# BigCiLeng/bilateral-driving

Hardware: AMD Instinct MI355X
Metric: train iters/sec (fwd+bwd) at 2M Gaussians, 6x1920x1080; HBM roofline % (higher is better)
Workload: dtype f32

## Files before the change

### bilateral_driving_amd/_lib.py

```python
from __future__ import annotations

import ctypes as C
import os
import threading

import torch

_HERE = os.path.dirname(os.path.abspath(__file__))
LIB_PATH = os.environ.get("BDS_LIB") or os.path.join(_HERE, "libbds.so")
ABI_VERSION = 6

_lock = threading.Lock()
_lib = None

_f = C.c_void_p
_i, _i64, _sz, _fl = C.c_int, C.c_int64, C.c_size_t, C.c_float


class BdsLevel(C.Structure):

    _fields_ = [("grid", C.c_void_p), ("v_grid", C.c_void_p), ("gx", C.c_int32), ("gy", C.c_int32), ("gl", C.c_int32),
                ("factor", C.c_int32), ("n_avg", C.c_int32)]


# ... 12 lines not shown
    "bds_abi_version": (C.c_int, []),
    "bds_strerror": (C.c_char_p, [_i]),
    "bds_set_option": (_i, [_i, _i]),
    "bds_get_option": (_i, [_i]),
    "bds_timer_create": (C.c_void_p, []),
    "bds_timer_destroy": (_i, [_f]),
    "bds_timer_mark": (_i, [_f, _f]),
    "bds_timer_elapsed_ms": (C.c_float, [_f, _f]),
    "bds_last_hip_error": (_i, []),
    "bds_sh_fwd": (_i, [_i64, _i, _i, _f, _f, _f, _f, _f]),
    "bds_sh_bwd": (_i, [_i64, _i, _i, _f, _f, _f, _f, _f, _f, _f]),
    "bds_project_fwd": (_i, [_i, _i64, _f, _f, _f, _f, _f, _f, _i, _i, _fl, _fl, _fl, _fl, _f, _f, _f, _f, _f, _f, _f]),
    "bds_project_bwd": (_i, [_i, _i64, _f, _f, _f, _f, _f, _i, _i, _fl, _f, _f, _f, _f, _f, _f, _f, _f, _f, _f, _f, _f]),
    "bds_isect_prepare_workspace_bytes": (_sz, [_i, _i64]),
    "bds_isect_visible_ids_offset": (_sz, [_i, _i64]),
    "bds_isect_build_workspace_bytes": (_sz, [_i, _i64, _i64]),
    "bds_isect_prepare": (_i, [_i, _i64, _f, _f, _f, _f, _f, _i, _i, _i, _f, _f, _sz, _i64, _i64, _f, _f, _i, _f]),
    "bds_isect_build": (_i, [_i, _i64, _i64, _i64, _f, _f, _f, _f, _f, _i, _i, _i, _f, _sz, _f, _sz, _f, _f, _f, _f, _i, _i, _f]),
    "bds_isect_tiles": (_i, [_i, _i64, _f, _f, _f, _f, _f, _i, _i, _i, _f, _f, _sz, _f, _sz, _i64, _f, _f, _f, C.POINTER(C.c_int64),
                             C.POINTER(C.c_int64), _f]),
    "bds_splat_pack_rgbd": (_i, [_i64, _f, _f, _f, _f, _f, _f, _f, _f, _f]),
    "bds_expected_depth_fwd": (_i, [_i64, _f, _f, _f, _f]),
    "bds_expected_depth_bwd": (_i, [_i64, _i, _i, _f, _f, _f, _f, _f, _f, _f]),
    "bds_expected_depth_split_fwd": (_i, [_i64, _i, _f, _f, _f, _f, _f]),
    "bds_expected_depth_split_bwd": (_i, [_i64, _i, _f, _f, _f, _f, _f, _f, _f, _f]),
    "bds_splat_pack": (_i, [_i64, _f, _i, _f, _f, _f, _f, _f, _f, _f, _f, _f, _i64, _f, _f]),
    "bds_rasterize_fwd": (_i, [_i, _i64, _i64, _f, _i, _f, _f, _i, _i, _i, _i, _i, _i, _f, _f, _f, _f, _f, _f, _f, _i, _i, _i64, _f]),
    "bds_rasterize_bwd": (_i, [_i, _i64, _i64, _f, _i, _f, _f, _i, _i, _i, _i, _i, _i, _f, _f, _f, _f, _f, _f, _f, _f, _i, _f, _i, _i, _i64, _f]),
    "bds_rasterize_kernel_name": (_i, [_i, _i, _i, _i, C.c_char_p, _i]),
    "bds_rasterize_bwd_schedule": (_i, [_i, _i, _i, _i, _i, _i, _i, _f, _f, _f, _f]),
    "bds_project_view_fwd": (_i, [_i, _i64, _f, _f, _f, _f, _f, _f, _i, _i, _fl, _fl, _fl, _fl, _f, _f, _f, _f, _f, _f, _f, _f, _f, _sz, _f, _f]),
    "bds_gaussian_block_bounds": (_i, [_i64, _f, _f, _f, _f]),
    "bds_sh_view_fwd": (_i, [_i64, _i, _i, _f, _f, _f, _f, _f, _f, _f, _f]),
    "bds_sh_view_bwd_list": (_i, [_i64, _f, _f, _i, _i, _f, _f, _f, _i, _f, _f, _f, _f, _i, _f]),
    "bds_splat_pack_sh": (_i, [_i64, _f, _f, _i, _i, _f, _f, _f, _f, _f, _f, _f, _f, _f, _f, _f, _f, _f, _i64, _f, _f]),
    "bds_nonfinite_flags": (_i, [_i, _f, _f, _f, _f, _f, _f]),
    "bds_project_view_bwd_list": (_i, [_i, _i64, _f, _f, _f, _f, _f, _f, _f, _f, _i, _i, _fl, _f, _f, _f, _f, _f, _f, _f, _f, _f, _f, _f]),
    "bds_view_grads_clear_list": (_i, [_i64, _f, _f, _i, _f, _f, _f, _f, _f, _f, _f, _f]),
    "bds_view_grads_add_list": (_i, [_i64, _f, _i, _f, _f, _f, _f, _f, _f, _f, _f, _f, _f, _f]),
    "bds_isect_counts_offset": (_sz, [_i]),
    "bds_rasterize_schedule_ints": (_i64, [_i, _i, _i]),
    "bds_rasterize_split_pool_ints": (_i64, [_i, _i, _i, _i, _i64, _i64]),
    "bds_rasterize_bwd_schedule_sort": (_i, [_i, _i, _i, _f, _f]),
    "bds_union_slots_workspace_bytes": (_sz, [_i64]),
    "bds_union_slots": (_i, [_i64, _f, _i64, _i, _f, _f, _f, _f, _f, _f, _f, _f, _sz, _f, _f, _f]),
    "bds_bilagrid_slice_fwd": (_i, [_i64, _f, _i, _i, _i, _f, _f, _f, _f]),
# ... 247 lines not shown
```

### bilateral_driving_amd/csrc/project.hip

```cpp
#include "bds_common.h"
#include "gs_math.h"

namespace bds {

constexpr int kProjBlock = 256;

template <bool kAA = false>
__global__ __launch_bounds__(kProjBlock) void project_fwd_kernel(
    int C, int64_t N, const float *__restrict__ means, const float *__restrict__ quats, const float *__restrict__ scales,
    const float *__restrict__ viewmats, const float *__restrict__ Ks, int W, int H, float eps2d, float near_plane,
    float far_plane, float radius_clip, int32_t *__restrict__ radii, float *__restrict__ means2d,
    float *__restrict__ depths, float *__restrict__ conics, float *__restrict__ comps,
    const float *__restrict__ opacities = nullptr, float *__restrict__ opac_eff = nullptr) {
  const int64_t g = (int64_t)blockIdx.x * kProjBlock + threadIdx.x;
  if (g >= N) return;
  float m[3] = {means[g * 3], means[g * 3 + 1], means[g * 3 + 2]};
  float q[4] = {quats[g * 4], quats[g * 4 + 1], quats[g * 4 + 2], quats[g * 4 + 3]};
  float s[3] = {scales[g * 3], scales[g * 3 + 1], scales[g * 3 + 2]};
  const float op = (kAA && opacities) ? opacities[g] : 0.f;
  for (int c = 0; c < C; c++) {
    Camera cam = load_camera(viewmats + c * 16, Ks + c * 9);
    Proj p = project_one(m, q, s, cam, W, H, eps2d, near_plane, far_plane, radius_clip, kAA);
    const int64_t o = (int64_t)c * N + g;
    radii[o] = p.radius;
// ... 63 lines not shown
    }
  }
  if (live) {
    for (int i = 0; i < 3; i++) { v_means[g * 3 + i] = am[i]; v_scales[g * 3 + i] = as[i]; }
    for (int i = 0; i < 4; i++) v_quats[g * 4 + i] = aq[i];
  }
}

template <bool kReduce, bool kAA = false>
__global__ __launch_bounds__(kProjBlock) void project_view_fwd_kernel(
    int64_t N, const float *__restrict__ means, const float *__restrict__ quats, const float *__restrict__ log_scales,
    const float *__restrict__ logits, const float *__restrict__ viewmat, const float *__restrict__ K, int W, int H,
    float eps2d, float near_plane, float far_plane, float radius_clip, float *__restrict__ scales,
    float *__restrict__ opacities, int32_t *__restrict__ radii, float *__restrict__ means2d, float *__restrict__ depths,
    float *__restrict__ conics, PrepReduceSlots rs, int32_t *__restrict__ tiles_per_gauss, int rows,
    const float *__restrict__ block_bounds, float *__restrict__ opac_eff = nullptr) {
  const int64_t g = (int64_t)blockIdx.x * kProjBlock + threadIdx.x;
  if (kReduce) {
    if (blockIdx.x == 0 && threadIdx.x == 0) *rs.m_total = 0;
    for (int64_t i = g; i < rs.zero_elems; i += (int64_t)gridDim.x * kProjBlock) rs.zero_me[i] = 0u;
  }
  if (block_bounds != nullptr) {
    const float *bb = block_bounds + (int64_t)blockIdx.x * 8;
    const float lo[3] = {bb[0], bb[1], bb[2]}, hi[3] = {bb[4], bb[5], bb[6]};
    if (!box_may_be_visible(lo, hi, bb[3], load_camera(viewmat, K), W, H, eps2d, near_plane, far_plane)) {
      if (g < N) {
        radii[g] = 0;
        scales[g * 3] = 0.f; scales[g * 3 + 1] = 0.f; scales[g * 3 + 2] = 0.f; opacities[g] = 0.f;
        if (rows) {
          float4 *row = reinterpret_cast<float4 *>(means2d + g * 8);
          row[0] = row[1] = make_float4(0.f, 0.f, 0.f, 0.f);
        } else {
          means2d[g * 2] = 0.f; means2d[g * 2 + 1] = 0.f;
          depths[g] = 0.f;
          conics[g * 3] = 0.f; conics[g * 3 + 1] = 0.f; conics[g * 3 + 2] = 0.f;
          if (kAA) opac_eff[g] = 0.f;
        }
        if (kReduce && tiles_per_gauss) tiles_per_gauss[g] = 0;
      }
      if (kReduce && threadIdx.x == 0) rs.sums256[blockIdx.x] = 0u;
      return;
    }
  }
  if (kReduce) {
    int radius = 0;
    if (g < N) {
      float m[3] = {means[g * 3], means[g * 3 + 1], means[g * 3 + 2]};
      float q[4] = {quats[g * 4], quats[g * 4 + 1], quats[g * 4 + 2], quats[g * 4 + 3]};
      float s[3];
#pragma unroll
      for (int k = 0; k < 3; k++) {
        s[k] = expf(log_scales[g * 3 + k]);
        scales[g * 3 + k] = s[k];
      }
      const float op = 1.f / (1.f + expf(-logits[g]));
// ... 4 lines not shown
      radii[g] = p.radius;
      const float oe = kAA ? op * p.comp : op;
      if (rows) {
        float4 *row = reinterpret_cast<float4 *>(means2d + g * 8);
        row[0] = make_float4(p.mx, p.my, p.depth, __int_as_float(p.radius));
        row[1] = make_float4(p.ca, p.cb, p.cc, oe);
      } else {
        means2d[g * 2] = p.mx; means2d[g * 2 + 1] = p.my;
        depths[g] = p.depth;
        conics[g * 3] = p.ca; conics[g * 3 + 1] = p.cb; conics[g * 3 + 2] = p.cc;
        if (kAA) opac_eff[g] = oe;
      }
      if (tiles_per_gauss) tiles_per_gauss[g] = 0;
    }
    const int cnt = __syncthreads_count(radius > 0);
    if (threadIdx.x == 0) rs.sums256[blockIdx.x] = (uint32_t)cnt;
    return;
  }
  if (g >= N) return;
  float m[3] = {means[g * 3], means[g * 3 + 1], means[g * 3 + 2]};
  float q[4] = {quats[g * 4], quats[g * 4 + 1], quats[g * 4 + 2], quats[g * 4 + 3]};
  float s[3];
#pragma unroll
  for (int k = 0; k < 3; k++) {
    s[k] = expf(log_scales[g * 3 + k]);
    scales[g * 3 + k] = s[k];
  }
  const float op = 1.f / (1.f + expf(-logits[g]));
  opacities[g] = op;
  Camera cam = load_camera(viewmat, K);
  Proj p = project_one(m, q, s, cam, W, H, eps2d, near_plane, far_plane, radius_clip, kAA);
  radii[g] = p.radius;
  const float oe = kAA ? op * p.comp : op;
// ... 197 lines not shown
  else
    hipLaunchKernelGGL(project_bwd_kernel<false>, dim3((unsigned)cdiv(N, kProjBlock)), dim3(kProjBlock), 0, as_stream(stream), C, N,
                       means, quats, scales, viewmats, Ks, W, H, eps2d, radii, v_means2d, v_depths, v_conics, v_means,
                       v_quats, v_scales, v_viewmats, static_cast<const float *>(nullptr));
  BDS_LAUNCH_CHECK();
  return BDS_OK;
}

static int view_rows(const float *means2d, const float *depths, const float *conics, int *rows) {
  const bool a = depths == means2d + 2, b = conics == means2d + 4;
  if (a != b || (a && !aligned16(means2d))) return BDS_EINVAL;
  *rows = a ? 1 : 0;
  return BDS_OK;
}

extern "C" int bds_project_view_fwd(int flags, int64_t N, const float *means, const float *quats, const float *log_scales,
                                    const float *logits, const float *viewmat, const float *K, int W, int H, float eps2d, float near_plane,
                                    float far_plane, float radius_clip, float *scales, float *opacities, float *opac_eff, int32_t *radii,
                                    float *means2d, float *depths, float *conics, int32_t *tiles_per_gauss, void *prep_ws,
                                    size_t prep_ws_bytes, const float *block_bounds, bds_stream_t stream) {
  BDS_REQUIRE((flags & ~BDS_PROJ_ANTIALIASED) == 0 && N >= 0 && W > 0 && H > 0);
  BDS_REQUIRE(prep_ws == nullptr || N > 0);
  if (N == 0) return BDS_OK;
  BDS_REQUIRE(means && quats && log_scales && logits && viewmat && K && scales && opacities && radii && means2d && depths && conics);
  int rows = 0;
  if (view_rows(means2d, depths, conics, &rows) != BDS_OK) return BDS_EINVAL;
  const bool aa = flags & BDS_PROJ_ANTIALIASED;
  BDS_REQUIRE(aa ? (rows || opac_eff) : opac_eff == nullptr);
  static_assert(kProjBlock == 256, "the tile stage reads the visible counts per 256 Gaussians");
  PrepReduceSlots rs{};
  if (prep_ws) {
    int rc = prep_reduce_slots(prep_ws, prep_ws_bytes, N, &rs);
    if (rc != BDS_OK) return rc;
  } else {
    tiles_per_gauss = nullptr;
  }
  const dim3 grid((unsigned)cdiv(N, kProjBlock)), block(kProjBlock);
#define BDS_VIEW_FWD(R, A)                                                                                                            \
  hipLaunchKernelGGL((project_view_fwd_kernel<R, A>), grid, block, 0, as_stream(stream), N, means, quats, log_scales, logits, viewmat, \
                     K, W, H, eps2d, near_plane, far_plane, radius_clip, scales, opacities, radii, means2d, depths, conics, rs,         \
                     tiles_per_gauss, rows, block_bounds, opac_eff)
  if (prep_ws) { if (aa) BDS_VIEW_FWD(true, true); else BDS_VIEW_FWD(true, false); }
  else         { if (aa) BDS_VIEW_FWD(false, true); else BDS_VIEW_FWD(false, false); }
#undef BDS_VIEW_FWD
  BDS_LAUNCH_CHECK();
  return BDS_OK;
}

namespace bds {
__global__ __launch_bounds__(kProjBlock) void block_bounds_kernel(int64_t N, const float *__restrict__ means,
                                                                 const float *__restrict__ log_scales, float *__restrict__ bounds) {
  __shared__ float red[kProjBlock / kWave][8];
  const int64_t g = (int64_t)blockIdx.x * kProjBlock + threadIdx.x;
  float v[7] = {3.0e38f, 3.0e38f, 3.0e38f, -3.0e38f, -3.0e38f, -3.0e38f, -3.0e38f};
  if (g < N) {
    for (int k = 0; k < 3; k++) { const float m = means[g * 3 + k]; v[k] = m; v[3 + k] = m; }
    v[6] = fmaxf(fmaxf(log_scales[g * 3], log_scales[g * 3 + 1]), log_scales[g * 3 + 2]);
    if (!(v[0] == v[0]) || !(v[1] == v[1]) || !(v[2] == v[2]) || !(v[6] == v[6])) {
      for (int k = 0; k < 3; k++) { v[k] = -3.0e38f; v[3 + k] = 3.0e38f; }
      v[6] = 80.f;
    }
// ... 91 lines not shown
```

### bilateral_driving_amd/csrc/tiles.hip

```cpp
#include "bds_common.h"
#include "gs_math.h"

namespace bds {

constexpr int kScanBlock = 256;
constexpr int kScanItems = 8;
constexpr int kScanTile = kScanBlock * kScanItems;

__device__ __forceinline__ uint32_t wave_incl_scan(uint32_t v) {
  const int lane = threadIdx.x & (kWave - 1);
#pragma unroll
  for (int o = 1; o < kWave; o <<= 1) {
    uint32_t t = __shfl_up(v, o);
    if (lane >= o) v += t;
  }
  return v;
}

__device__ __forceinline__ uint32_t block_excl_scan(uint32_t v, uint32_t &total, uint32_t *lds_w ) {
  const int lane = threadIdx.x & (kWave - 1), wv = threadIdx.x / kWave;
  const int nw = blockDim.x / kWave;
  uint32_t inc = wave_incl_scan(v);
  if (lane == kWave - 1) lds_w[wv] = inc;
  __syncthreads();
// ... 713 lines not shown
  if (threadIdx.x == 0) tile_sums[blockIdx.x] = tot;
}

constexpr int kCompactSpan = kScanTile / kShortChunk + 1;
struct VisCompactSh {
  uint32_t lw[kScanBlock / kWave + 1];
  uint32_t h[kCompactSpan][256];
};
__device__ __forceinline__ void visible_compact_block(VisCompactSh &sh, int vb, int nvb, int64_t CN, const int32_t *radii, const float *depths,
                                                      const uint32_t *tile_sums, uint32_t *keys, uint32_t *vals, uint32_t *hist,
                                                      uint32_t *ghist, uint64_t *n_vis_out, uint32_t *asc, int compact, int sums_per_tile,
                                                      int sd) {
  constexpr int kSpan = kCompactSpan;
  uint32_t *lw = sh.lw;
  auto &h = sh.h;
#pragma unroll
  for (int t = 0; t < kSpan; t++) h[t][threadIdx.x] = 0;
  uint32_t part = 0;
  for (int b = threadIdx.x; b < vb * sums_per_tile; b += kScanBlock) part += tile_sums[b];
  uint32_t my_offset;
  block_excl_scan(part, my_offset, lw);
  const int64_t base = (int64_t)vb * kScanTile + (int64_t)threadIdx.x * kScanItems;
  bool vis[kScanItems];
  uint32_t s = 0;
#pragma unroll
  for (int i = 0; i < kScanItems; i++) {
    vis[i] = base + i < CN && radii[base + i] > 0;
    s += vis[i] ? 1u : 0u;
  }
  uint32_t tot;
  uint32_t j = block_excl_scan(s, tot, lw) + my_offset;
  const uint32_t chunk0 = my_offset >> kChunkShift;
#pragma unroll
  for (int i = 0; i < kScanItems; i++) {
    if (vis[i]) {
      const uint32_t key = __float_as_uint(depths[(base + i) * sd]);
// ... 299 lines not shown
  if (ws_bytes < L.bytes) return BDS_EWORKSPACE;
  out->sums256 = L.temp;
  out->zero_me = L.tables;
  out->zero_elems = (int64_t)short_sort_elems(CN);
  out->m_total = L.total;
  return BDS_OK;
}

extern "C" size_t bds_isect_visible_ids_offset(int C, int64_t N) {
  if (C < 1 || N < 0) return 0;
  char *const base = reinterpret_cast<char *>(static_cast<uintptr_t>(4096));
  const PrepWs L = prep_layout(base, (int64_t)C * N);
  return static_cast<size_t>(reinterpret_cast<char *>(L.asc) - base);
}

extern "C" size_t bds_isect_prepare_workspace_bytes(int C, int64_t N) {
  if (C < 1 || N < 0) return 0;
  return prep_layout(nullptr, (int64_t)C * N).bytes;
}

extern "C" size_t bds_isect_build_workspace_bytes(int C, int64_t N, int64_t M) {
  (void)C; (void)N;
  if (M < 0) return 0;
  return build_layout(nullptr, M).bytes;
}

constexpr int kCountMEff = 2, kCountVisEff = 3, kCountOverflow = 4;
__global__ __launch_bounds__(256) void finish_counts_kernel(const uint32_t *__restrict__ btot, int nblocks, uint64_t *__restrict__ counts_dev,
                                                           volatile int64_t *__restrict__ counts_host, int64_t cap_m, int64_t cap_vis) {
  __shared__ unsigned long long part[256];
// ... 267 lines not shown
```

### bilateral_driving_amd/fused_view.py

```python
from __future__ import annotations

import contextlib
import ctypes as C
import math
import os
import weakref
from typing import Dict, Optional, Sequence

import torch
from torch import Tensor

from . import _lib as L
from . import gs_ops as ops
from .bilagrid import _levels_struct

TILE = 16
LIST_TILE = int(os.environ.get("BDS_LIST_TILE", "64"))
SH_IN_PACK = os.environ.get("BDS_SH_IN_PACK", "0") == "1"
SH_IN_PACK_DEV = os.environ.get("BDS_SH_IN_PACK_DEV", "1") == "1"


_PROJ_ROWS = os.environ.get("BDS_PROJ_ROWS", "1") == "1"


# ... 65 lines not shown

    def __getitem__(self, k):
        if k in self._LAZY and not dict.__contains__(self, k):
            g = dict.__getitem__(self, "_rgb_g_raw").detach().clamp(max=1.0)
            if k == "original_rgb":
                g = g + dict.__getitem__(self, "_sky").detach() * (1.0 - dict.__getitem__(self, "opacity").detach())
            dict.__setitem__(self, k, g)
        return dict.__getitem__(self, k)

    def __contains__(self, k):
        return k in self._LAZY or dict.__contains__(self, k)


class _Front:
    pass


class _Lists:
    pass


SPLIT_POOL_PER_TILE = int(os.environ.get("BDS_SPLIT_POOL_PER_TILE", "4096"))


def _split(cfg: dict, list_tile: int, n_tiles: int, have_schedule: bool):
    if list_tile <= TILE or not have_schedule:
        return 0, 0, 0
    n = int(cfg.get("split_len") or os.environ.get("BDS_SPLIT_LEN", "0"))
    if n <= 0:
        return 0, 0, 0
# ... 17 lines not shown
    return _front_finish(_front_begin(cfg, means, quats, log_scales, logits, sh, viewmat), before_wait)


def _front_begin(cfg: dict, means, quats, log_scales, logits, sh, viewmat) -> _Front:
    sh_rest = None
    if isinstance(sh, (tuple, list)):
        sh, sh_rest = sh[0].contiguous(), sh[1].contiguous()
        assert sh.dim() == 2 and sh.shape[1] == 3 and sh_rest.dim() == 3 and sh_rest.shape[2] == 3 and cfg.get("caps") is None
    L.require_gpu(means, quats, log_scales, logits, sh, viewmat)
    lib, st = L.lib(), L.stream()
    dev = means.device
    W, H = cfg["width"], cfg["height"]
    N, K = means.shape[0], (sh.shape[1] if sh_rest is None else 1 + sh_rest.shape[1])
    means, quats, log_scales, logits, sh = (t.contiguous() for t in (means, quats, log_scales, logits, sh))
    viewmat, Kmat = viewmat.contiguous(), cfg["K"].contiguous()
    scales, opac = _empty((N, 3), dev), _empty((N,), dev)
    radii = _empty((1, N), dev, torch.int32)
    caps = cfg.get("caps")
    in_pack = cfg.get("sh_in_pack", SH_IN_PACK if caps is None else SH_IN_PACK_DEV)
    pack_colours = sh_rest is not None or (in_pack and (K * 3) % 4 == 0 and sh.data_ptr() % 16 == 0)
    aa = bool(cfg.get("antialiased"))
    opac_eff = None
    if pack_colours and _PROJ_ROWS and N > 0:
        rows = _empty((N, 8), dev)
        means2d, depths, conics, opac_row = rows[None, :, 0:2], rows[None, :, 2], rows[None, :, 4:7], rows[:, 7]
    else:
        means2d, depths, conics, opac_row = _empty((1, N, 2), dev), _empty((1, N), dev), _empty((1, N, 3), dev), opac
        if aa:
            opac_row = opac_eff = _empty((N,), dev)
    tiles_per_gauss = _empty((1, N), dev, torch.int32)
    ws_bytes = lib.bds_isect_prepare_workspace_bytes(1, N)
    ws = cfg.get("prep_ws")
    if ws is None:
        ws = _empty((max(ws_bytes, 16),), dev, torch.uint8)
    assert ws.dtype == torch.uint8 and ws.is_contiguous() and ws.numel() >= ws_bytes and ws.device == dev
    pre_reduced = False
    bounds = cfg.get("block_bounds")
    with L.timed("project_fwd"):
        args = (L.PROJ_ANTIALIASED if aa else 0, N, L.ptr(means), L.ptr(quats), L.ptr(log_scales), L.ptr(logits), L.ptr(viewmat),
                L.ptr(Kmat), W, H, cfg["eps2d"], cfg["near_plane"], cfg["far_plane"], cfg["radius_clip"], L.ptr(scales), L.ptr(opac),
                L.ptr(opac_eff), L.ptr(radii), _dp(means2d), _dp(depths), _dp(conics))
        if caps is not None and N > 0:
            rc = lib.bds_project_view_fwd(*args, L.ptr(tiles_per_gauss), L.ptr(ws), ws_bytes, L.ptr(bounds), st)
            pre_reduced = rc == L.BDS_OK
            if rc != L.BDS_ECAPACITY:
                L.check(rc, "bds_project_view_fwd")
        if not pre_reduced:
            L.check(lib.bds_project_view_fwd(*args, None, None, 0, L.ptr(bounds), st), "bds_project_view_fwd")
    f = _Front()
    f.list_tile = cfg.get("list_tile", LIST_TILE)
    f.lists = _lists_begin(means2d, radii, depths, (_dp(conics), _dp(opac_row)) if cfg["tile_cull"] else None, W, H, f.list_tile, caps,
                           ws, ws_bytes, tiles_per_gauss, pre_reduced)
    cam_pos = cfg["cam_pos"].contiguous()
    if pack_colours:
        sh_rgb, colors = None, None
    else:
        sh_rgb, colors = _empty((N, 3), dev), _empty((1, N, 4), dev)
    f.cfg = cfg
    f.means, f.quats, f.log_scales, f.sh, f.viewmat, f.cam_pos = means, quats, log_scales, sh, viewmat, cam_pos
    f.sh_rest, f.K = sh_rest, K
    f.scales, f.opac, f.radii, f.means2d, f.depths, f.conics = scales, opac, radii, means2d, depths, conics
    f.opac_row = opac_row
    f.aa = aa
# ... 500 lines not shown
               grid_grads: Optional[Sequence[Tensor]] = None, after_forward=None, **kwargs):
    from .losses import _PhotometricTV, photometric_tv_train, slots_value
    cam_pos = kwargs.pop("cam_pos", None)
    if cam_pos is None:
        cam_pos = torch.linalg.inv(viewmat.detach())[:3, 3].contiguous()
    grad_arena, arena_rows = kwargs.pop("grad_arena", None), int(kwargs.pop("arena_rows", 0))
    grad_sink = kwargs.pop("grad_sink", None)
    list_tile, caps = kwargs.pop("list_tile", None), kwargs.pop("caps", None)
    prep_ws, two_phase = kwargs.pop("prep_ws", None), bool(kwargs.pop("two_phase", False))
    g2d_buf = kwargs.pop("g2d_buf", None)
    tail_buf, defer_pose_sum = kwargs.pop("tail_buf", None), bool(kwargs.pop("defer_pose_sum", False))
    lazy_loss = bool(kwargs.pop("lazy_loss", False))
    defer_epilogue = bool(kwargs.pop("defer_epilogue", True))
    split_len, split_cap = kwargs.pop("split_len", None), kwargs.pop("split_cap", None)
    block_bounds = kwargs.pop("block_bounds", None)
    row_catchup = kwargs.pop("row_catchup", None)
    tv_grids, tv_grid_grads = kwargs.pop("tv_grids", None), kwargs.pop("tv_grid_grads", None)
    opts = dict(sh_degree=3, near_plane=0.1, far_plane=1e10, radius_clip=0.0, eps2d=0.3, tile_cull=True, antialiased=False)
    opts.update({k: kwargs.pop(k) for k in list(kwargs) if k in opts})
    assert not kwargs, f"unknown arguments {sorted(kwargs)}"
    cfg = dict(width=int(width), height=int(height), K=K, cam_pos=cam_pos.detach(), factors=tuple(int(f) for f in factors),
               sh_degree=int(opts["sh_degree"]), near_plane=float(opts["near_plane"]), far_plane=float(opts["far_plane"]),
               radius_clip=float(opts["radius_clip"]), eps2d=float(opts["eps2d"]), tile_cull=bool(opts["tile_cull"]),
               grad_arena=grad_arena, grad_sink=grad_sink, img_idx=None if img_idx is None else int(img_idx), arena_rows=arena_rows,
               list_tile=int(LIST_TILE if list_tile is None else list_tile), caps=caps, prep_ws=prep_ws, g2d_buf=g2d_buf, tail_buf=tail_buf,
               defer_epilogue=defer_epilogue, split_len=split_len, split_cap=split_cap, block_bounds=block_bounds,
               defer_pose_sum=defer_pose_sum, row_catchup=row_catchup, antialiased=bool(opts["antialiased"]))
    gs = [g if g.dim() == 5 else g[None] for g in grids]
    if grad_arena is not None and (arena_rows >= 1 or grad_sink is not None):
        cfg["grids_in_place"] = all(g.grad is not None and grad_arena.get(f"grid{i}") is not None
                                    and g.grad.data_ptr() == grad_arena[f"grid{i}"].data_ptr() for i, g in enumerate(gs))
    if (grid_grads is not None and _LOSS_IN_TRANSFORM and not _LOSS_TWO_STEP and all(g.requires_grad and g.is_contiguous() for g in gs)
            and all(a.is_contiguous() and a.numel() == g.numel() for a, g in zip(grid_grads, gs)) and target.is_contiguous()
            and target.dtype == torch.float32 and tuple(target.shape) == (int(height), int(width), 3) and target.data_ptr() % 16 == 0):
        from .losses import _levels_struct as _tv_levels
        tvg = gs if tv_grids is None else [g if g.dim() == 5 else g[None] for g in tv_grids]
        tvgg = list(grid_grads) if tv_grid_grads is None else list(tv_grid_grads)
        cfg["train_loss"] = dict(target=target, grids=tvg, grid_grads=tvgg, levels=_tv_levels(tvg, tvgg, [1] * len(tvg)),
                                 weights=(C.c_float * max(len(tvg), 1))(*[float(w) for w in tv_weights]))
    names = ("means", "quats", "log_scales", "opacity_logits", "sh")
    leaves = [params[k] for k in names]
    needs = (False, *[bool(t.requires_grad) for t in leaves], bool(sky.requires_grad), bool(viewmat.requires_grad),
# ... 64 lines not shown
```

### bilateral_driving_amd/graph_slots.py

```python
from __future__ import annotations

import ctypes as C
from typing import Optional

import torch
from torch import Tensor

from . import _lib as L
from . import harness as Hn
from .fused_view import ListCapacity


class ViewGraph:

    def __init__(self, graph, out, caps: ListCapacity, prep_ws: Tensor, sky: Tensor, viewmat: Tensor, graph_bwd, graph_tail=None):
        self.graph, self.graph_bwd, self.graph_tail, self.out, self.caps, self.prep_ws = graph, graph_bwd, graph_tail, out, caps, prep_ws
        self._loss_slots = out.get("loss_slots")
        self.rgb, self.depth, self.opacity = out["rgb"], out["depth"], out["opacity"]
        self.v_sky, self.v_viewmat = sky.grad, viewmat.grad
        self.done, self.fwd_done = torch.cuda.Event(), torch.cuda.Event()

    @property
    def loss(self) -> Tensor:
        from .losses import slots_value
        torch.cuda.current_stream(self._loss_slots.device).wait_event(self.done)
        return slots_value(self._loss_slots)


def camera_centre(viewmat: Tensor) -> Tensor:
    vm = viewmat.detach()
    return -(vm[:3, :3].transpose(0, 1) @ vm[:3, 3]).contiguous()


BLOCK_BOUNDS = __import__("os").environ.get("BDS_BLOCK_BOUNDS", "1") == "1"
GRAD_ROWS = __import__("os").environ.get("BDS_GRAD_ROWS", "1") == "1"
SPLIT_LIST_LEN = int(__import__("os").environ.get("BDS_SPLIT_LIST_LEN", "6144"))


def split_len_for(info):
    if SPLIT_LIST_LEN <= 0:
        return 0, 0
    offs = info["isect_offsets"].reshape(-1).long()
    if offs.numel() < 2:
        return 0, 0
    M = int(info["n_isects"])
    lens = torch.diff(offs, append=offs.new_tensor([M]))
    longest, mean = int(lens.max()), float(lens.float().mean())
    if not (longest >= SPLIT_LIST_LEN and longest >= 4.0 * mean):
        return 0, 0
# ... 141 lines not shown
```

### bilateral_driving_amd/graph_view.py

```python
from __future__ import annotations

from typing import Dict, List, Optional, Sequence

import torch
from torch import Tensor

from . import _lib as L
from .dist import ROW_NAMES, FlatGradients
from .fused_view import LIST_TILE
from . import harness as Hn
from .graph_slots import BLOCK_BOUNDS, GRAD_ROWS, FrameCapacities, ViewGraph, camera_centre as _camera_centre


class FrameGraph(FrameCapacities):
    def __init__(self, params: Dict[str, Tensor], cams: Sequence[Hn.Camera], grids: Sequence[Tensor], skies: Sequence[Tensor],
                 targets: Sequence[Tensor], factors: Sequence[int] = Hn.FACTORS_3, tv_weight: float = 0.01,
                 img_indices: Optional[Sequence[int]] = None, headroom: float = 1.5, list_tile: Optional[int] = None,
                 sh_degree: int = 3, extra_params: Sequence[Tensor] = (), overlap: bool = True, exchange=None, dynamic: bool = False,
                 calib_cams: Optional[Sequence[Hn.Camera]] = None, clear_grads: bool = True, row_catchup=None, antialiased: bool = False):
        assert sorted(params.keys()) == sorted(ROW_NAMES), "params: means, quats, log_scales, opacity_logits, sh"
        self._ctor = dict(cams=cams, grids=grids, skies=skies, targets=targets, factors=factors, tv_weight=tv_weight, img_indices=img_indices,
                          headroom=headroom, list_tile=list_tile, sh_degree=sh_degree, extra_params=extra_params, overlap=overlap,
                          exchange=exchange, dynamic=dynamic, calib_cams=calib_cams, clear_grads=clear_grads, row_catchup=row_catchup)
        self.params = {k: params[k] for k in ROW_NAMES}
        self.grids = list(grids)
        self.V = len(cams)
# ... 47 lines not shown
        self.n_captures = 0
        self._reprovision = False
        lib = L.lib()
        self._ws_bytes = int(lib.bds_isect_prepare_workspace_bytes(1, self.N))
        self._ids_off = int(lib.bds_isect_visible_ids_offset(1, self.N))
        self._nvis_off = int(lib.bds_isect_counts_offset(3))
        self.prep_ws = [torch.zeros(max(self._ws_bytes, 16), device=self.dev, dtype=torch.uint8) for _ in range(self.V)]
        self.g2d = [torch.zeros(2, self.N, 2, device=self.dev, dtype=torch.float32) for _ in range(self.V)] if self.fx is None else None
        self._tail_rows = L.POSE_GRAD_SLOTS + L.LOSS_SLOTS * L.LOSS_SLOT_STRIDE // L.GRAD_RECORD_FLOATS
        self._tails = torch.zeros(self.V, self._tail_rows, L.GRAD_RECORD_FLOATS, device=self.dev, dtype=torch.float32)
        self._vm = torch.zeros(self.V, 4, 4, device=self.dev, dtype=torch.float32)
        self._defer_pose = self.fx is None and all(c.viewmat.requires_grad for c in self.cams)
        self._unions = [0] * self.V
        self.split_len, self.split_cap = [0] * self.V, [0] * self.V
        self._bounds = torch.zeros((self.N + 255) // 256, 8, device=self.dev) if BLOCK_BOUNDS and self.N > 0 else None
        self.calibrate()
        self.capture()

    def _view_kwargs(self, v: int) -> dict:
        kw = dict(factors=self.factors, tv_weight=self.tv_weight, caps=self.caps[v], prep_ws=self.prep_ws[v], list_tile=self.list_tile,
                  sh_degree=self.sh_degree, two_phase=True, lazy_loss=True, split_len=self.split_len[v], split_cap=self.split_cap[v],
                  defer_epilogue=not self.overlap, block_bounds=self._bounds, row_catchup=self.row_catchup, antialiased=self.antialiased)
        if self.fx is not None:
            kw.update(grad_sink=self.fx.static_sink(v), grid_grads=None)
            if self.dynamic:
                kw.update(grid_grads=self.sel_grads[v], grad_arena={f"grid{i}": g for i, g in enumerate(self.sel_grads[v])},
                          tv_grids=self.grids, tv_grid_grads=[self.arena[f"grid{i}"] for i in range(len(self.grids))])
        else:
            grid_grads = [self.arena[f"grid{i}"] for i in range(len(self.grids))]
            arena = self.arena
            if self.dynamic:
                arena = dict(self.arena, **{f"grid{i}": g for i, g in enumerate(self.sel_grads[v])})
                kw.update(tv_grids=self.grids, tv_grid_grads=grid_grads)
                grid_grads = self.sel_grads[v]
            kw.update(grid_grads=grid_grads, grad_arena=arena, arena_rows=1 if v == 0 else 2, g2d_buf=self.g2d[v])
            if self._defer_pose:
                kw.update(tail_buf=self._tails[v], defer_pose_sum=True)
# ... 54 lines not shown
        from .dist import _active
        if self.coll or _active():
            return torch.cuda.graph(graph, pool=pool, capture_error_mode="thread_local")
        return torch.cuda.graph(graph, pool=pool)

    def _reset_static_grads(self) -> None:
        for v in range(self.V):
            self.skies[v].grad = None
            self.cams[v].viewmat.grad = self._vm[v] if self._defer_pose else None

    def capture(self) -> None:
        self.views = [None] * self.V
        self.begin_graph = self.begin_graph_rest = None
        self._reprovision = False
        torch.cuda.synchronize()
        if self.fx is not None:
            self.fx.static_setup(self._unions)
        self._point_grads_at_flat()
        self._reset_static_grads()
        side = torch.cuda.Stream(device=self.dev)
        side.wait_stream(torch.cuda.current_stream(self.dev))
        with torch.cuda.stream(side):
            self._frame_begin()
            self._begin_body()
            for v in range(self.V):
                out = self._phase_fwd(v)
                if self.fx is not None:
                    self.fx.static_begin_view(v, out["union_mask"])
                self._phase_bwd(v, out, tail=False)
                if self.fx is not None:
# ... 124 lines not shown
```

### include/bds.h

```cpp
#ifndef BDS_H
#define BDS_H

#include <stddef.h>
#include <stdint.h>

#ifdef __cplusplus
extern "C" {
#endif

#define BDS_ABI_VERSION 6

#define BDS_OK 0
#define BDS_EINVAL (-1)
#define BDS_EWORKSPACE (-2)
#define BDS_ELAUNCH (-3)
#define BDS_ECAPACITY (-4)

typedef void *bds_stream_t;

int bds_abi_version(void);
const char *bds_strerror(int code);

int bds_set_option(int which, int value);
int bds_get_option(int which);
// ... 9 lines not shown
int bds_sh_bwd(int64_t n, int K, int deg, const float *dirs, const float *coeffs, const uint8_t *masks,
               const float *v_out, float *v_coeffs, float *v_dirs, bds_stream_t stream);

int bds_project_fwd(int C, int64_t N, const float *means, const float *quats, const float *scales, const float *opacities,
                    const float *viewmats, const float *Ks, int W, int H, float eps2d, float near_plane, float far_plane,
                    float radius_clip, int32_t *radii, float *means2d, float *depths, float *conics, float *compensations,
                    float *opac_eff, bds_stream_t stream);
int bds_project_bwd(int C, int64_t N, const float *means, const float *quats, const float *scales,
                    const float *viewmats, const float *Ks, int W, int H, float eps2d, const int32_t *radii,
                    const float *conics, const float *compensations, const float *v_means2d, const float *v_depths,
                    const float *v_conics, const float *v_compensations, float *v_means, float *v_quats,
                    float *v_scales, float *v_viewmats, bds_stream_t stream);

size_t bds_isect_prepare_workspace_bytes(int C, int64_t N);
size_t bds_isect_visible_ids_offset(int C, int64_t N);
size_t bds_isect_build_workspace_bytes(int C, int64_t N, int64_t M);
int bds_isect_prepare(int C, int64_t N, const float *means2d, const int32_t *radii, const float *depths,
                      const float *conics, const float *opacities, int tile_size, int tile_w, int tile_h,
                      int32_t *tiles_per_gauss, void *ws, size_t ws_bytes, int64_t M_capacity, int64_t n_visible_capacity,
                      int64_t *counts, void *event, int compact, bds_stream_t stream);
int bds_isect_build(int C, int64_t N, int64_t M, int64_t n_visible, const float *means2d, const int32_t *radii,
                    const float *depths,
                    const float *conics, const float *opacities, int tile_size, int tile_w, int tile_h, const void *ws,
                    size_t ws_bytes, void *ws2,
                    size_t ws2_bytes, int64_t *isect_ids, int32_t *flatten_ids, int32_t *isect_offsets,
                    int32_t *visible_ids, int device_counts, int compact, bds_stream_t stream);
int bds_isect_tiles(int C, int64_t N, const float *means2d, const int32_t *radii, const float *depths,
                    const float *conics, const float *opacities, int tile_size, int tile_w, int tile_h,
                    int32_t *tiles_per_gauss, void *ws, size_t ws_bytes, void *ws2, size_t ws2_bytes,
                    int64_t flatten_capacity, int64_t *isect_ids, int32_t *flatten_ids, int32_t *isect_offsets,
// ... 72 lines not shown
                           bds_stream_t stream);

#define BDS_LOSS_SLOT_STRIDE 64
int bds_l1_tv_train(int64_t n, const float *a, const float *b, int nlevels, const bds_bilagrid_level_t *levels, const float *weights,
                    float v_loss, float *loss_out, int loss_slots, float *v_a, bds_stream_t stream);

int bds_gaussian_block_bounds(int64_t N, const float *means, const float *log_scales, float *block_bounds, bds_stream_t stream);
#define BDS_PROJ_ACCUMULATE 1
#define BDS_PROJ_ACTIVATED 2
#define BDS_PROJ_ANTIALIASED 4
int bds_project_view_fwd(int flags, int64_t N, const float *means, const float *quats, const float *log_scales, const float *logits,
                         const float *viewmat, const float *K, int W, int H, float eps2d, float near_plane, float far_plane,
                         float radius_clip, float *scales, float *opacities, float *opac_eff, int32_t *radii, float *means2d,
                         float *depths, float *conics, int32_t *tiles_per_gauss, void *prep_ws, size_t prep_ws_bytes,
                         const float *block_bounds, bds_stream_t stream);
int bds_sh_view_fwd(int64_t N, int K, int degrees_to_use, const float *means, const float *cam_pos, const float *coeffs,
                    const int32_t *radii, const float *depths, float *sh_rgb, float *colors, bds_stream_t stream);
#define BDS_POSE_GRAD_SLOTS 64
int bds_sh_view_bwd_list(int64_t n_list, const uint64_t *n_dev, const int32_t *ids, int K, int degrees_to_use, const float *means,
                         const float *cam_pos, const float *sh_rgb, int sh_rgb_by_rank, const float *v_records, float *v_coeffs,
                         float *v_coeffs_rest, const int32_t *row_map, int accumulate, bds_stream_t stream);
int bds_nonfinite_flags(int n_tensors, const float *const *tensors, const int64_t *counts, const int *kinds, uint32_t *flags_dev,
                        uint32_t *flags_pinned, bds_stream_t stream);
int bds_project_view_bwd_list(int flags, int64_t n_list, const uint64_t *n_dev, const int32_t *ids, const float *means,
                              const float *quats, const float *scales, const float *opacities, const float *viewmat, const float *K,
                              int W, int H, float eps2d, const float *v_records, float *v_means, float *v_quats, float *v_scales,
                              float *v_opacities, float *v_colors, float *v_viewmat_slots, float *grad2d, float *absgrad2d,
                              const int32_t *row_map, bds_stream_t stream);
int bds_view_grads_clear_list(int64_t n_list, const uint64_t *n_dev, const int32_t *ids, int K, float *v_means, float *v_quats,
                              float *v_log_scales, float *v_logits, float *v_sh, float *grad2d, float *absgrad2d, bds_stream_t stream);
// ... 219 lines not shown
```

Baseline: 1078.

## Keep per-view front buffers persistent and skip rewriting already-zeroed culled blocks

Per-view forward output buffers (scales, opacities, radii, rows, tiles) are now reused across iterations via a FrontBuffers cache. A per-block state word records whether a frustum-culled block's outputs are already zeroed, so later iterations skip the zero stores for blocks that stay culled. The compact-scan kernel also returns early for scan tiles with no visible entries, skipping histogram init and the visibility pass. This saves write bandwidth for off-screen Gaussians. The cost is persistent memory per view and state that must be reset whenever buffers are reallocated or graphs recaptured.

```diff
diff --git a/bilateral_driving_amd/_lib.py b/bilateral_driving_amd/_lib.py
--- a/bilateral_driving_amd/_lib.py
+++ b/bilateral_driving_amd/_lib.py
@@ -50,6 +50,7 @@
     "bds_project_bwd": (_i, [_i, _i64, _f, _f, _f, _f, _f, _i, _i, _fl, _f, _f, _f, _f, _f, _f, _f, _f, _f, _f, _f, _f]),
     "bds_isect_prepare_workspace_bytes": (_sz, [_i, _i64]),
     "bds_isect_visible_ids_offset": (_sz, [_i, _i64]),
+    "bds_isect_block_counts_offset": (_sz, [_i, _i64]),
     "bds_isect_build_workspace_bytes": (_sz, [_i, _i64, _i64]),
     "bds_isect_prepare": (_i, [_i, _i64, _f, _f, _f, _f, _f, _i, _i, _i, _f, _f, _sz, _i64, _i64, _f, _f, _i, _f]),
     "bds_isect_build": (_i, [_i, _i64, _i64, _i64, _f, _f, _f, _f, _f, _i, _i, _i, _f, _sz, _f, _sz, _f, _f, _f, _f, _i, _i, _f]),
@@ -66,6 +67,7 @@
     "bds_rasterize_kernel_name": (_i, [_i, _i, _i, _i, C.c_char_p, _i]),
     "bds_rasterize_bwd_schedule": (_i, [_i, _i, _i, _i, _i, _i, _i, _f, _f, _f, _f]),
     "bds_project_view_fwd": (_i, [_i, _i64, _f, _f, _f, _f, _f, _f, _i, _i, _fl, _fl, _fl, _fl, _f, _f, _f, _f, _f, _f, _f, _f, _f, _sz, _f, _f]),
+    "bds_project_view_fwd_kept": (_i, [_i, _i64, _f, _f, _f, _f, _f, _f, _i, _i, _fl, _fl, _fl, _fl, _f, _f, _f, _f, _f, _f, _f, _f, _f, _sz, _f, _f, _f]),
     "bds_gaussian_block_bounds": (_i, [_i64, _f, _f, _f, _f]),
     "bds_sh_view_fwd": (_i, [_i64, _i, _i, _f, _f, _f, _f, _f, _f, _f, _f]),
     "bds_sh_view_bwd_list": (_i, [_i64, _f, _f, _i, _i, _f, _f, _f, _i, _f, _f, _f, _f, _i, _f]),
diff --git a/bilateral_driving_amd/csrc/project.hip b/bilateral_driving_amd/csrc/project.hip
--- a/bilateral_driving_amd/csrc/project.hip
+++ b/bilateral_driving_amd/csrc/project.hip
@@ -101,7 +101,7 @@
     float eps2d, float near_plane, float far_plane, float radius_clip, float *__restrict__ scales,
     float *__restrict__ opacities, int32_t *__restrict__ radii, float *__restrict__ means2d, float *__restrict__ depths,
     float *__restrict__ conics, PrepReduceSlots rs, int32_t *__restrict__ tiles_per_gauss, int rows,
-    const float *__restrict__ block_bounds, float *__restrict__ opac_eff = nullptr) {
+    const float *__restrict__ block_bounds, float *__restrict__ opac_eff = nullptr, uint32_t *__restrict__ block_state = nullptr) {
   const int64_t g = (int64_t)blockIdx.x * kProjBlock + threadIdx.x;
   if (kReduce) {
     if (blockIdx.x == 0 && threadIdx.x == 0) *rs.m_total = 0;
@@ -111,7 +111,8 @@
     const float *bb = block_bounds + (int64_t)blockIdx.x * 8;
     const float lo[3] = {bb[0], bb[1], bb[2]}, hi[3] = {bb[4], bb[5], bb[6]};
     if (!box_may_be_visible(lo, hi, bb[3], load_camera(viewmat, K), W, H, eps2d, near_plane, far_plane)) {
-      if (g < N) {
+      const bool kept = block_state != nullptr && block_state[blockIdx.x] == 1u;
+      if (g < N && !kept) {
         radii[g] = 0;
         scales[g * 3] = 0.f; scales[g * 3 + 1] = 0.f; scales[g * 3 + 2] = 0.f; opacities[g] = 0.f;
         if (rows) {
@@ -126,6 +127,10 @@
         if (kReduce && tiles_per_gauss) tiles_per_gauss[g] = 0;
       }
       if (kReduce && threadIdx.x == 0) rs.sums256[blockIdx.x] = 0u;
+      if (block_state != nullptr && !kept) {
+        __syncthreads();
+        if (threadIdx.x == 0) block_state[blockIdx.x] = 1u;
+      }
       return;
     }
   }
@@ -160,9 +165,13 @@
       if (tiles_per_gauss) tiles_per_gauss[g] = 0;
     }
     const int cnt = __syncthreads_count(radius > 0);
-    if (threadIdx.x == 0) rs.sums256[blockIdx.x] = (uint32_t)cnt;
+    if (threadIdx.x == 0) {
+      rs.sums256[blockIdx.x] = (uint32_t)cnt;
+      if (block_state != nullptr) block_state[blockIdx.x] = 0u;
+    }
     return;
   }
+  if (block_state != nullptr && threadIdx.x == 0) block_state[blockIdx.x] = 0u;
   if (g >= N) return;
   float m[3] = {means[g * 3], means[g * 3 + 1], means[g * 3 + 2]};
   float q[4] = {quats[g * 4], quats[g * 4 + 1], quats[g * 4 + 2], quats[g * 4 + 3]};
@@ -390,13 +399,14 @@
   return BDS_OK;
 }
 
-extern "C" int bds_project_view_fwd(int flags, int64_t N, const float *means, const float *quats, const float *log_scales,
-                                    const float *logits, const float *viewmat, const float *K, int W, int H, float eps2d, float near_plane,
-                                    float far_plane, float radius_clip, float *scales, float *opacities, float *opac_eff, int32_t *radii,
-                                    float *means2d, float *depths, float *conics, int32_t *tiles_per_gauss, void *prep_ws,
-                                    size_t prep_ws_bytes, const float *block_bounds, bds_stream_t stream) {
+static int project_view_fwd(int flags, int64_t N, const float *means, const float *quats, const float *log_scales, const float *logits,
+                            const float *viewmat, const float *K, int W, int H, float eps2d, float near_plane, float far_plane,
+                            float radius_clip, float *scales, float *opacities, float *opac_eff, int32_t *radii, float *means2d,
+                            float *depths, float *conics, int32_t *tiles_per_gauss, void *prep_ws, size_t prep_ws_bytes,
+                            const float *block_bounds, uint32_t *block_state, bds_stream_t stream) {
   BDS_REQUIRE((flags & ~BDS_PROJ_ANTIALIASED) == 0 && N >= 0 && W > 0 && H > 0);
   BDS_REQUIRE(prep_ws == nullptr || N > 0);
+  BDS_REQUIRE(block_state == nullptr || block_bounds != nullptr);
   if (N == 0) return BDS_OK;
   BDS_REQUIRE(means && quats && log_scales && logits && viewmat && K && scales && opacities && radii && means2d && depths && conics);
   int rows = 0;
@@ -415,12 +425,34 @@
 #define BDS_VIEW_FWD(R, A)                                                                                                            \
   hipLaunchKernelGGL((project_view_fwd_kernel<R, A>), grid, block, 0, as_stream(stream), N, means, quats, log_scales, logits, viewmat, \
                      K, W, H, eps2d, near_plane, far_plane, radius_clip, scales, opacities, radii, means2d, depths, conics, rs,         \
-                     tiles_per_gauss, rows, block_bounds, opac_eff)
+                     tiles_per_gauss, rows, block_bounds, opac_eff, block_state)
   if (prep_ws) { if (aa) BDS_VIEW_FWD(true, true); else BDS_VIEW_FWD(true, false); }
   else         { if (aa) BDS_VIEW_FWD(false, true); else BDS_VIEW_FWD(false, false); }
 #undef BDS_VIEW_FWD
   BDS_LAUNCH_CHECK();
   return BDS_OK;
+}
+
+extern "C" int bds_project_view_fwd(int flags, int64_t N, const float *means, const float *quats, const float *log_scales,
+                                    const float *logits, const float *viewmat, const float *K, int W, int H, float eps2d, float near_plane,
+                                    float far_plane, float radius_clip, float *scales, float *opacities, float *opac_eff, int32_t *radii,
+                                    float *means2d, float *depths, float *conics, int32_t *tiles_per_gauss, void *prep_ws,
+                                    size_t prep_ws_bytes, const float *block_bounds, bds_stream_t stream) {
+  return project_view_fwd(flags, N, means, quats, log_scales, logits, viewmat, K, W, H, eps2d, near_plane, far_plane, radius_clip, scales,
+                          opacities, opac_eff, radii, means2d, depths, conics, tiles_per_gauss, prep_ws, prep_ws_bytes, block_bounds,
+                          nullptr, stream);
+}
+
+extern "C" int bds_project_view_fwd_kept(int flags, int64_t N, const float *means, const float *quats, const float *log_scales,
+                                         const float *logits, const float *viewmat, const float *K, int W, int H, float eps2d,
+                                         float near_plane, float far_plane, float radius_clip, float *scales, float *opacities,
+                                         float *opac_eff, int32_t *radii, float *means2d, float *depths, float *conics,
+                                         int32_t *tiles_per_gauss, void *prep_ws, size_t prep_ws_bytes, const float *block_bounds,
+                                         uint32_t *block_state, bds_stream_t stream) {
+  BDS_REQUIRE(block_state != nullptr && block_bounds != nullptr);
+  return project_view_fwd(flags, N, means, quats, log_scales, logits, viewmat, K, W, H, eps2d, near_plane, far_plane, radius_clip, scales,
+                          opacities, opac_eff, radii, means2d, depths, conics, tiles_per_gauss, prep_ws, prep_ws_bytes, block_bounds,
+                          block_state, stream);
 }
 
 namespace bds {
diff --git a/bilateral_driving_amd/csrc/tiles.hip b/bilateral_driving_amd/csrc/tiles.hip
--- a/bilateral_driving_amd/csrc/tiles.hip
+++ b/bilateral_driving_amd/csrc/tiles.hip
@@ -751,12 +751,23 @@
   constexpr int kSpan = kCompactSpan;
   uint32_t *lw = sh.lw;
   auto &h = sh.h;
-#pragma unroll
-  for (int t = 0; t < kSpan; t++) h[t][threadIdx.x] = 0;
   uint32_t part = 0;
   for (int b = threadIdx.x; b < vb * sums_per_tile; b += kScanBlock) part += tile_sums[b];
   uint32_t my_offset;
   block_excl_scan(part, my_offset, lw);
+  const uint32_t per_sum = (uint32_t)(kScanTile / sums_per_tile);
+  const int n_sums = (int)(((uint32_t)CN + per_sum - 1u) / per_sum);
+  uint32_t own = 0;
+  for (int k = 0; k < sums_per_tile; k++) {
+    const int b = vb * sums_per_tile + k;
+    if (b < n_sums) own += tile_sums[b];
+  }
+  if (own == 0) {
+    if (vb == nvb - 1 && threadIdx.x == 0) *n_vis_out = (uint64_t)my_offset;
+    return;
+  }
+#pragma unroll
+  for (int t = 0; t < kSpan; t++) h[t][threadIdx.x] = 0;
   const int64_t base = (int64_t)vb * kScanTile + (int64_t)threadIdx.x * kScanItems;
   bool vis[kScanItems];
   uint32_t s = 0;
@@ -1086,6 +1097,13 @@
   return static_cast<size_t>(reinterpret_cast<char *>(L.asc) - base);
 }
 
+extern "C" size_t bds_isect_block_counts_offset(int C, int64_t N) {
+  if (C < 1 || N < 0) return 0;
+  char *const base = reinterpret_cast<char *>(static_cast<uintptr_t>(4096));
+  const PrepWs L = prep_layout(base, (int64_t)C * N);
+  return static_cast<size_t>(reinterpret_cast<char *>(L.temp) - base);
+}
+
 extern "C" size_t bds_isect_prepare_workspace_bytes(int C, int64_t N) {
   if (C < 1 || N < 0) return 0;
   return prep_layout(nullptr, (int64_t)C * N).bytes;
diff --git a/bilateral_driving_amd/fused_view.py b/bilateral_driving_amd/fused_view.py
--- a/bilateral_driving_amd/fused_view.py
+++ b/bilateral_driving_amd/fused_view.py
@@ -103,6 +103,45 @@
 
 class _Front:
     pass
+
+
+class FrontBuffers:
+
+    def __init__(self):
+        self.tensors, self.state, self._i = [], None, 0
+
+    @staticmethod
+    def _not_capturing() -> None:
+        if torch.cuda.is_current_stream_capturing():
+            raise L.BdsError("FrontBuffers: new buffers inside a stream capture (run the slot's forward once outside the capture first)")
+
+    def begin(self):
+        self._i = 0
+        return self._take
+
+    def _take(self, shape, dev, dtype=torch.float32) -> Tensor:
+        i, self._i = self._i, self._i + 1
+        t = self.tensors[i] if i < len(self.tensors) else None
+        if t is None or tuple(t.shape) != tuple(shape) or t.dtype != dtype or t.device != dev:
+            self._not_capturing()
+            del self.tensors[i:]
+            t = torch.empty(shape, device=dev, dtype=dtype)
+            self.tensors.append(t)
+            self.state = None
+        return t
+
+    def end(self, N: int) -> Tensor:
+        if len(self.tensors) > self._i:
+            del self.tensors[self._i:]
+            self.state = None
+        if self.state is None:
+            self._not_capturing()
+            self.state = torch.zeros((N + 255) // 256, device=self.tensors[0].device, dtype=torch.int32)
+        return self.state
+
+    def reset(self) -> None:
+        if self.state is not None:
+            self.state.zero_()
 
 
 class _Lists:
@@ -150,21 +189,24 @@
     N, K = means.shape[0], (sh.shape[1] if sh_rest is None else 1 + sh_rest.shape[1])
     means, quats, log_scales, logits, sh = (t.contiguous() for t in (means, quats, log_scales, logits, sh))
     viewmat, Kmat = viewmat.contiguous(), cfg["K"].contiguous()
-    scales, opac = _empty((N, 3), dev), _empty((N,), dev)
-    radii = _empty((1, N), dev, torch.int32)
+    keep = cfg.get("front_bufs") if N > 0 and cfg.get("block_bounds") is not None else None
+    out_buf = keep.begin() if keep is not None else _empty
+    scales, opac = out_buf((N, 3), dev), out_buf((N,), dev)
+    radii = out_buf((1, N), dev, torch.int32)
     caps = cfg.get("caps")
     in_pack = cfg.get("sh_in_pack", SH_IN_PACK if caps is None else SH_IN_PACK_DEV)
     pack_colours = sh_rest is not None or (in_pack and (K * 3) % 4 == 0 and sh.data_ptr() % 16 == 0)
     aa = bool(cfg.get("antialiased"))
     opac_eff = None
     if pack_colours and _PROJ_ROWS and N > 0:
-        rows = _empty((N, 8), dev)
+        rows = out_buf((N, 8), dev)
         means2d, depths, conics, opac_row = rows[None, :, 0:2], rows[None, :, 2], rows[None, :, 4:7], rows[:, 7]
     else:
-        means2d, depths, conics, opac_row = _empty((1, N, 2), dev), _empty((1, N), dev), _empty((1, N, 3), dev), opac
+        means2d, depths, conics, opac_row = out_buf((1, N, 2), dev), out_buf((1, N), dev), out_buf((1, N, 3), dev), opac
         if aa:
-            opac_row = opac_eff = _empty((N,), dev)
-    tiles_per_gauss = _empty((1, N), dev, torch.int32)
+            opac_row = opac_eff = out_buf((N,), dev)
+    tiles_per_gauss = out_buf((1, N), dev, torch.int32)
+    keep_state = keep.end(N) if keep is not None else None
     ws_bytes = lib.bds_isect_prepare_workspace_bytes(1, N)
     ws = cfg.get("prep_ws")
     if ws is None:
@@ -176,13 +218,17 @@
         args = (L.PROJ_ANTIALIASED if aa else 0, N, L.ptr(means), L.ptr(quats), L.ptr(log_scales), L.ptr(logits), L.ptr(viewmat),
                 L.ptr(Kmat), W, H, cfg["eps2d"], cfg["near_plane"], cfg["far_plane"], cfg["radius_clip"], L.ptr(scales), L.ptr(opac),
                 L.ptr(opac_eff), L.ptr(radii), _dp(means2d), _dp(depths), _dp(conics))
+        def project(*tile_stage):
+            if keep is None:
+                return lib.bds_project_view_fwd(*args, *tile_stage, L.ptr(bounds), st)
+            return lib.bds_project_view_fwd_kept(*args, *tile_stage, L.ptr(bounds), L.ptr(keep_state), st)
         if caps is not None and N > 0:
-            rc = lib.bds_project_view_fwd(*args, L.ptr(tiles_per_gauss), L.ptr(ws), ws_bytes, L.ptr(bounds), st)
+            rc = project(L.ptr(tiles_per_gauss), L.ptr(ws), ws_bytes)
             pre_reduced = rc == L.BDS_OK
             if rc != L.BDS_ECAPACITY:
                 L.check(rc, "bds_project_view_fwd")
         if not pre_reduced:
-            L.check(lib.bds_project_view_fwd(*args, None, None, 0, L.ptr(bounds), st), "bds_project_view_fwd")
+            L.check(project(None, None, 0), "bds_project_view_fwd")
     f = _Front()
     f.list_tile = cfg.get("list_tile", LIST_TILE)
     f.lists = _lists_begin(means2d, radii, depths, (_dp(conics), _dp(opac_row)) if cfg["tile_cull"] else None, W, H, f.list_tile, caps,
@@ -713,6 +759,7 @@
     defer_epilogue = bool(kwargs.pop("defer_epilogue", True))
     split_len, split_cap = kwargs.pop("split_len", None), kwargs.pop("split_cap", None)
     block_bounds = kwargs.pop("block_bounds", None)
+    front_bufs = kwargs.pop("front_bufs", None)
     row_catchup = kwargs.pop("row_catchup", None)
     tv_grids, tv_grid_grads = kwargs.pop("tv_grids", None), kwargs.pop("tv_grid_grads", None)
     opts = dict(sh_degree=3, near_plane=0.1, far_plane=1e10, radius_clip=0.0, eps2d=0.3, tile_cull=True, antialiased=False)
@@ -724,7 +771,7 @@
                grad_arena=grad_arena, grad_sink=grad_sink, img_idx=None if img_idx is None else int(img_idx), arena_rows=arena_rows,
                list_tile=int(LIST_TILE if list_tile is None else list_tile), caps=caps, prep_ws=prep_ws, g2d_buf=g2d_buf, tail_buf=tail_buf,
                defer_epilogue=defer_epilogue, split_len=split_len, split_cap=split_cap, block_bounds=block_bounds,
-               defer_pose_sum=defer_pose_sum, row_catchup=row_catchup, antialiased=bool(opts["antialiased"]))
+               front_bufs=front_bufs, defer_pose_sum=defer_pose_sum, row_catchup=row_catchup, antialiased=bool(opts["antialiased"]))
     gs = [g if g.dim() == 5 else g[None] for g in grids]
     if grad_arena is not None and (arena_rows >= 1 or grad_sink is not None):
         cfg["grids_in_place"] = all(g.grad is not None and grad_arena.get(f"grid{i}") is not None
diff --git a/bilateral_driving_amd/graph_slots.py b/bilateral_driving_amd/graph_slots.py
--- a/bilateral_driving_amd/graph_slots.py
+++ b/bilateral_driving_amd/graph_slots.py
@@ -33,6 +33,7 @@
 
 
 BLOCK_BOUNDS = __import__("os").environ.get("BDS_BLOCK_BOUNDS", "1") == "1"
+BLOCK_KEEP = __import__("os").environ.get("BDS_BLOCK_KEEP", "1") == "1"
 GRAD_ROWS = __import__("os").environ.get("BDS_GRAD_ROWS", "1") == "1"
 SPLIT_LIST_LEN = int(__import__("os").environ.get("BDS_SPLIT_LIST_LEN", "6144"))
 
diff --git a/bilateral_driving_amd/graph_view.py b/bilateral_driving_amd/graph_view.py
--- a/bilateral_driving_amd/graph_view.py
+++ b/bilateral_driving_amd/graph_view.py
@@ -7,9 +7,9 @@
 
 from . import _lib as L
 from .dist import ROW_NAMES, FlatGradients
-from .fused_view import LIST_TILE
+from .fused_view import LIST_TILE, FrontBuffers
 from . import harness as Hn
-from .graph_slots import BLOCK_BOUNDS, GRAD_ROWS, FrameCapacities, ViewGraph, camera_centre as _camera_centre
+from .graph_slots import BLOCK_BOUNDS, BLOCK_KEEP, GRAD_ROWS, FrameCapacities, ViewGraph, camera_centre as _camera_centre
 
 
 class FrameGraph(FrameCapacities):
@@ -87,13 +87,15 @@
         self._unions = [0] * self.V
         self.split_len, self.split_cap = [0] * self.V, [0] * self.V
         self._bounds = torch.zeros((self.N + 255) // 256, 8, device=self.dev) if BLOCK_BOUNDS and self.N > 0 else None
+        self.front_bufs = [FrontBuffers() for _ in range(self.V)] if BLOCK_KEEP and self._bounds is not None else None
         self.calibrate()
         self.capture()
 
     def _view_kwargs(self, v: int) -> dict:
         kw = dict(factors=self.factors, tv_weight=self.tv_weight, caps=self.caps[v], prep_ws=self.prep_ws[v], list_tile=self.list_tile,
                   sh_degree=self.sh_degree, two_phase=True, lazy_loss=True, split_len=self.split_len[v], split_cap=self.split_cap[v],
-                  defer_epilogue=not self.overlap, block_bounds=self._bounds, row_catchup=self.row_catchup, antialiased=self.antialiased)
+                  defer_epilogue=not self.overlap, block_bounds=self._bounds, row_catchup=self.row_catchup, antialiased=self.antialiased,
+                  front_bufs=None if self.front_bufs is None else self.front_bufs[v])
         if self.fx is not None:
             kw.update(grad_sink=self.fx.static_sink(v), grid_grads=None)
             if self.dynamic:
@@ -178,6 +180,8 @@
         self.begin_graph = self.begin_graph_rest = None
         self._reprovision = False
         torch.cuda.synchronize()
+        for fb in self.front_bufs or ():
+            fb.reset()
         if self.fx is not None:
             self.fx.static_setup(self._unions)
         self._point_grads_at_flat()
diff --git a/include/bds.h b/include/bds.h
--- a/include/bds.h
+++ b/include/bds.h
@@ -47,6 +47,7 @@
 
 size_t bds_isect_prepare_workspace_bytes(int C, int64_t N);
 size_t bds_isect_visible_ids_offset(int C, int64_t N);
+size_t bds_isect_block_counts_offset(int C, int64_t N);
 size_t bds_isect_build_workspace_bytes(int C, int64_t N, int64_t M);
 int bds_isect_prepare(int C, int64_t N, const float *means2d, const int32_t *radii, const float *depths,
                       const float *conics, const float *opacities, int tile_size, int tile_w, int tile_h,
@@ -149,6 +150,11 @@
                          float radius_clip, float *scales, float *opacities, float *opac_eff, int32_t *radii, float *means2d,
                          float *depths, float *conics, int32_t *tiles_per_gauss, void *prep_ws, size_t prep_ws_bytes,
                          const float *block_bounds, bds_stream_t stream);
+int bds_project_view_fwd_kept(int flags, int64_t N, const float *means, const float *quats, const float *log_scales, const float *logits,
+                              const float *viewmat, const float *K, int W, int H, float eps2d, float near_plane, float far_plane,
+                              float radius_clip, float *scales, float *opacities, float *opac_eff, int32_t *radii, float *means2d,
+                              float *depths, float *conics, int32_t *tiles_per_gauss, void *prep_ws, size_t prep_ws_bytes,
+                              const float *block_bounds, uint32_t *block_state, bds_stream_t stream);
 int bds_sh_view_fwd(int64_t N, int K, int degrees_to_use, const float *means, const float *cam_pos, const float *coeffs,
                     const int32_t *radii, const float *depths, float *sh_rgb, float *colors, bds_stream_t stream);
 #define BDS_POSE_GRAD_SLOTS 64
```

After: 1096, median of 6. +1.7%, better.
